# SamsungLabs/Metis

Measured on AMD Instinct MI355X. Metric: best_plan_iter_time_ms, lower is better.
Workload: dtype bf16; 1 GPU; model=gpt3-2.7b, global_batch=16, seq_len=2048, parallelism=dp1_tp1_pp1, microbatch=16

## Files before the change

### metis_amd/ops/hip/bindings.cpp

```cpp
#include <torch/extension.h>

#include <vector>

std::vector<torch::Tensor> layernorm_fwd(
    torch::Tensor x, torch::Tensor gamma, torch::Tensor beta, double eps);
std::vector<torch::Tensor> layernorm_bwd(
    torch::Tensor dy, torch::Tensor x, torch::Tensor gamma,
    torch::Tensor mean, torch::Tensor rstd);
std::vector<torch::Tensor> bias_residual_layernorm_fwd(
    torch::Tensor y, torch::Tensor bias, torch::Tensor residual,
    torch::Tensor gamma, torch::Tensor beta, double eps);
torch::Tensor bias_residual_add(
    torch::Tensor y, torch::Tensor bias, torch::Tensor residual);
std::vector<torch::Tensor> layernorm_bwd_add(
    torch::Tensor dy, torch::Tensor dres, torch::Tensor x, torch::Tensor gamma,
    torch::Tensor mean, torch::Tensor rstd, bool want_colsum);
std::vector<torch::Tensor> gelu_tanh_bwd_bgrad(torch::Tensor h, torch::Tensor da);
void adamw_step(
    torch::Tensor master, torch::Tensor model, torch::Tensor grad,
    torch::Tensor m, torch::Tensor v,
    double lr, double beta1, double beta2, double eps,
    double weight_decay, long step, double grad_scale);
torch::Tensor attn_decode(
    torch::Tensor q, torch::Tensor k, torch::Tensor v, double scale);
torch::Tensor attn_decode_ragged(
    torch::Tensor q, torch::Tensor k, torch::Tensor v, torch::Tensor kv_lens,
    double scale, long num_splits);
torch::Tensor attn_decode_ragged_fp8(
    torch::Tensor q, torch::Tensor k8, torch::Tensor v8,
    torch::Tensor k_scale, torch::Tensor v_scale, torch::Tensor kv_lens,
    double scale, long num_splits);
void kv_quant_store(
    torch::Tensor k, torch::Tensor v, torch::Tensor k8, torch::Tensor v8,
    torch::Tensor k_scale, torch::Tensor v_scale, torch::Tensor slots,
    torch::Tensor pos);
torch::Tensor w8_linear(
    torch::Tensor x, torch::Tensor w8, torch::Tensor scale,
    c10::optional<torch::Tensor> bias, long num_splits);
long w8_linear_auto_splits(long N, long K);
torch::Tensor ce_row_max(torch::Tensor logits);
torch::Tensor ce_row_sumexp(torch::Tensor logits, torch::Tensor m);
std::vector<torch::Tensor> qkv_rope_split(
    torch::Tensor qkv, long nq, long nkv, long head_dim,
    torch::Tensor cos_t, torch::Tensor sin_t);
torch::Tensor qkv_rope_split_bwd(
    torch::Tensor dq, torch::Tensor dk, torch::Tensor dv, long head_dim,
    torch::Tensor cos_t, torch::Tensor sin_t);
torch::Tensor lt_fp8_matmul(
    torch::Tensor x, torch::Tensor w,
    torch::Tensor scale_x, torch::Tensor scale_w);
std::vector<torch::Tensor> lt_fc1_forward(
    torch::Tensor x, torch::Tensor w, torch::Tensor bias);
std::vector<torch::Tensor> lt_matmul_dgelu_bgrad(
    torch::Tensor dy, torch::Tensor w2, torch::Tensor pre_gelu);
std::vector<torch::Tensor> attn_fwd(
    torch::Tensor q, torch::Tensor k, torch::Tensor v, double scale);
std::vector<torch::Tensor> attn_bwd(
    torch::Tensor q, torch::Tensor k, torch::Tensor v,
    torch::Tensor d_o, torch::Tensor lse, torch::Tensor delta,
    double scale);
torch::Tensor attn_bwd_delta(torch::Tensor o, torch::Tensor d_o);
std::vector<torch::Tensor> attn_fwd_packed(
    torch::Tensor qkv, long H, long Hkv, long D, double scale);
torch::Tensor attn_bwd_delta_packed(torch::Tensor o, torch::Tensor d_o, long H);
torch::Tensor attn_bwd_packed(
    torch::Tensor qkv, torch::Tensor d_o, torch::Tensor lse, torch::Tensor delta,
    long H, long Hkv, long D, double scale);
torch::Tensor gemm_bf16(
    torch::Tensor a, torch::Tensor b_nk, c10::optional<torch::Tensor> bias,
    long epilogue);
torch::Tensor mfma_tile_probe(torch::Tensor a, torch::Tensor b);
torch::Tensor gemm8_bf16(torch::Tensor x, torch::Tensor w);
std::vector<torch::Tensor> rmsnorm_fwd(
    torch::Tensor x, torch::Tensor gamma, double eps);
std::vector<torch::Tensor> rmsnorm_bwd(
    torch::Tensor dy, torch::Tensor x, torch::Tensor gamma, torch::Tensor rstd);
torch::Tensor rope_apply(
    torch::Tensor x, torch::Tensor cos_t, torch::Tensor sin_t, bool backward);
torch::Tensor swiglu_fwd(torch::Tensor a, torch::Tensor b);
std::vector<torch::Tensor> swiglu_bwd(
    torch::Tensor dy, torch::Tensor a, torch::Tensor b);
std::vector<torch::Tensor> cross_entropy_fwd(
    torch::Tensor logits, torch::Tensor labels);
torch::Tensor cross_entropy_bwd(
    torch::Tensor logits, torch::Tensor labels, torch::Tensor lse,
    torch::Tensor grad_scale);
std::vector<torch::Tensor> qkv_split_transpose(
    torch::Tensor qkv, long nq, long nkv, long head_dim);
torch::Tensor qkv_split_transpose_bwd(
    torch::Tensor dq, torch::Tensor dk, torch::Tensor dv, long head_dim);
torch::Tensor heads_merge(torch::Tensor x);
torch::Tensor heads_unmerge(torch::Tensor y, long H);
torch::Tensor tr16_probe(long stride_elems);
torch::Tensor lt_linear_dgrad_tn(torch::Tensor dy, torch::Tensor wt);
torch::Tensor lt_linear_dgrad(torch::Tensor dy, torch::Tensor w, long algo);
torch::Tensor lt_linear_wgrad(torch::Tensor dy, torch::Tensor x, long algo);
long lt_version();
std::vector<long> lt_supported_algos(
    const std::string& op, long M, long N, long K);
long lt_heuristic_algo(const std::string& op, long M, long N, long K);
long lt_wgrad_bgradb_algos(long M, long N, long K);
torch::Tensor transpose_bf16(torch::Tensor w);
void transpose_bf16_out(torch::Tensor w, torch::Tensor wt);

PYBIND11_MODULE(TORCH_EXTENSION_NAME, m) {
    m.def("layernorm_fwd", &layernorm_fwd,
          "fused LayerNorm forward (bf16, fp32 stats)");
    m.def("layernorm_bwd", &layernorm_bwd,
          "fused LayerNorm backward (dx + dgamma/dbeta)");
    m.def("bias_residual_layernorm_fwd", &bias_residual_layernorm_fwd,
          "x = residual + (y + bias) with both bf16 roundings, then "
          "LayerNorm(x) -> (x, z, mean, rstd)");
    m.def("bias_residual_add", &bias_residual_add,
          "x = residual + (y + bias) with both bf16 roundings");
    m.def("layernorm_bwd_add", &layernorm_bwd_add,
          "LayerNorm backward with a residual gradient folded in -> "
          "(g = dres + dx, dgamma, dbeta, colsum of g in fp32 or empty)");
    m.def("gelu_tanh_bwd_bgrad", &gelu_tanh_bwd_bgrad,
          "tanh-GeLU backward -> (dh bf16, dbias = column sums of dh, fp32)");
    m.def("adamw_step", &adamw_step, "fused AdamW step");
    m.def("attn_fwd", &attn_fwd,
          "flash attention forward (causal, GQA) -> (O, LSE)");
    m.def("attn_bwd", &attn_bwd,
          "flash attention backward -> (dQ, dK_per_head, dV_per_head)");
    m.def("attn_bwd_delta", &attn_bwd_delta,
          "rowsum(dO * O) in fp32 -> [B,H,S] (contiguous bf16 inputs)");
    m.def("attn_fwd_packed", &attn_fwd_packed,
          "flash attention forward on qkv [B,S,(H+2Hkv)D] in place "
          "(H == Hkv) -> (O [B,S,H*D], LSE [B,H,S])");
    m.def("attn_bwd_delta_packed", &attn_bwd_delta_packed,
          "rowsum(dO * O) of [B,S,H*D] operands in fp32 -> [B,H,S]");
    m.def("attn_bwd_packed", &attn_bwd_packed,
          "flash attention backward on qkv in place -> dqkv [B,S,(H+2Hkv)D]");
    m.def("gemm_bf16", &gemm_bf16,
          "MFMA bf16 GEMM A[M,K] @ B[N,K]^T with fused epilogue "
          "(0=none, 1=bias, 2=bias+gelu)");
    m.def("gemm8_bf16", &gemm8_bf16,
          "256^2-tile 2-buffer glds bf16 GEMM x[M,K] @ w[N,K]^T");
    m.def("mfma_tile_probe", &mfma_tile_probe,
          "single-wave 16x16x32 MFMA layout probe");
    m.def("rmsnorm_fwd", &rmsnorm_fwd, "fused RMSNorm forward");
    m.def("rmsnorm_bwd", &rmsnorm_bwd, "fused RMSNorm backward");
    m.def("rope_apply", &rope_apply, "rotary embedding (fwd/bwd by flag)");
    m.def("swiglu_fwd", &swiglu_fwd, "fused silu(a)*b");
    m.def("swiglu_bwd", &swiglu_bwd, "fused SwiGLU backward");
    m.def("cross_entropy_fwd", &cross_entropy_fwd,
          "fused CE over bf16 logits -> (per-row loss, lse)");
    m.def("cross_entropy_bwd", &cross_entropy_bwd,
          "fused CE backward -> bf16 dlogits");
    m.def("qkv_split_transpose", &qkv_split_transpose,
          "[B,S,(nq+2nkv)D] -> q/k/v [B,h,S,D] in one pass");
    m.def("qkv_split_transpose_bwd", &qkv_split_transpose_bwd,
          "dq/dk/dv -> fused dqkv layout");
    m.def("heads_merge", &heads_merge, "[B,H,S,D] -> [B,S,H*D]");
    m.def("heads_unmerge", &heads_unmerge, "[B,S,H*D] -> [B,H,S,D]");
    m.def("attn_decode", &attn_decode,
          "single-query attention over cached K/V (GQA, online softmax)");
    m.def("attn_decode_ragged", &attn_decode_ragged,
          "ragged split-S single-query attention over a padded K/V cache "
          "(per-row kv_lens, strided views, GQA group per workgroup)",
          pybind11::arg("q"), pybind11::arg("k"), pybind11::arg("v"),
          pybind11::arg("kv_lens"), pybind11::arg("scale"),
          pybind11::arg("num_splits") = 0);
    m.def("attn_decode_ragged_fp8", &attn_decode_ragged_fp8,
          "ragged split-S single-query attention over an fp8 (e4m3fn) K/V "
          "cache with one fp32 scale per (batch row, kv head, position)",
          pybind11::arg("q"), pybind11::arg("k8"), pybind11::arg("v8"),
          pybind11::arg("k_scale"), pybind11::arg("v_scale"),
          pybind11::arg("kv_lens"), pybind11::arg("scale"),
          pybind11::arg("num_splits") = 0);
    m.def("kv_quant_store", &kv_quant_store,
          "quantise bf16 K/V rows [N,Hkv,T,D] to e4m3fn + per-row fp32 scale "
          "and store them at position pos[n] + t of cache row slots[n]",
          pybind11::arg("k"), pybind11::arg("v"), pybind11::arg("k8"),
          pybind11::arg("v8"), pybind11::arg("k_scale"),
          pybind11::arg("v_scale"), pybind11::arg("slots"),
          pybind11::arg("pos"));
    m.def("w8_linear", &w8_linear,
          "fp8 (e4m3fn) weight-only linear for 1 <= M <= 16 bf16 rows: "
          "scale[n] * (x @ w8^T) + bias, fp32 accumulation, split-K",
          pybind11::arg("x"), pybind11::arg("w8"), pybind11::arg("scale"),
          pybind11::arg("bias") = pybind11::none(),
          pybind11::arg("num_splits") = 0);
    m.def("w8_linear_auto_splits", &w8_linear_auto_splits,
          "split count w8_linear picks for num_splits = 0 (from N and K only)");
    m.def("ce_row_max", &ce_row_max, "per-row max of bf16 logits (fp32)");
    m.def("ce_row_sumexp", &ce_row_sumexp,
          "per-row sum(exp(x - m)) of bf16 logits (fp32)");
    m.def("qkv_rope_split", &qkv_rope_split,
          "fused QKV relayout + RoPE (neox) forward");
    m.def("qkv_rope_split_bwd", &qkv_rope_split_bwd,
          "fused QKV relayout + RoPE backward gather");
    m.def("lt_fp8_matmul", &lt_fp8_matmul,
          "fp8 e4m3 GEMM with per-tensor scales, bf16 out");
    m.def("lt_fc1_forward", &lt_fc1_forward,
          "hipblaslt GEMM with GELU_AUX_BIAS epilogue (fc1 fused)");
    m.def("lt_matmul_dgelu_bgrad", &lt_matmul_dgelu_bgrad,
          "hipblaslt GEMM with DGELU_BGRAD epilogue (fc2 data grad fused)");
    m.def("lt_linear_dgrad_tn", &lt_linear_dgrad_tn,
          "dx [M,K] = dy [M,N] @ wt [K,N]^T (hipBLASLt TN route)");
    m.def("lt_linear_dgrad", &lt_linear_dgrad,
          "dx [M,K] = dy [M,N] @ w [N,K]; algo = solution index or -1");
    m.def("lt_linear_wgrad", &lt_linear_wgrad,
          "dw [N,K] = dy [M,N]^T @ x [M,K]; algo = solution index or -1");
    m.def("lt_version", &lt_version, "hipblasLtGetVersion");
    m.def("lt_supported_algos", &lt_supported_algos,
          "supported solution indices for op (dgrad_tn|dgrad|wgrad) at M,N,K");
    m.def("lt_heuristic_algo", &lt_heuristic_algo,
          "solution index of the heuristic's first choice");
    m.def("lt_wgrad_bgradb_algos", &lt_wgrad_bgradb_algos,
          "number of weight-gradient algorithms with the BGRADB epilogue");
    m.def("transpose_bf16", &transpose_bf16, "wt [C,R] = w [R,C]^T");
    m.def("transpose_bf16_out", &transpose_bf16_out,
          "transpose into an existing [C,R] buffer");
    m.def("tr16_probe", &tr16_probe,
          "ds_read_b64_tr_b16 lane-semantics probe (debug)");
}
```

### metis_amd/ops/hip/lt_gemm.cpp

```cpp

#include <torch/extension.h>

#include <hipblaslt/hipblaslt.h>
#include <hipblaslt/hipblaslt-ext.hpp>

#include <c10/hip/HIPStream.h>

#include <climits>
#include <mutex>
#include <stdexcept>
#include <string>
#include <unordered_map>
#include <vector>

namespace {

#define LT_CHECK(expr)                                                        \
    do {                                                                      \
        hipblasStatus_t s_ = (expr);                                          \
        TORCH_CHECK(s_ == HIPBLAS_STATUS_SUCCESS, "hipblaslt error ",         \
                    (int)s_, " at ", #expr);                                  \
    } while (0)

hipblasLtHandle_t lt_handle() {
    static hipblasLtHandle_t handle = [] {
        hipblasLtHandle_t h;
        LT_CHECK(hipblasLtCreate(&h));
        return h;
    }();
    return handle;
}

constexpr size_t kWorkspaceBytes = 64ull << 20;

torch::Tensor workspace(const torch::TensorOptions& opt) {
    static torch::Tensor ws;
    if (!ws.defined() || ws.numel() < (long)kWorkspaceBytes)
        ws = torch::empty({(long)kWorkspaceBytes},
                          opt.dtype(torch::kUInt8));
    return ws;
}

struct LtPlan {
    hipblasLtMatmulDesc_t desc{};
    hipblasLtMatrixLayout_t a{}, b{}, d{};
    hipblasLtMatmulAlgo_t algo{};
    bool has_algo = false;
};

std::unordered_map<std::string, LtPlan>& plan_cache() {
    static std::unordered_map<std::string, LtPlan> cache;
    return cache;
}
std::mutex cache_mutex;

void destroy_plan(LtPlan& plan) {
    if (plan.a) hipblasLtMatrixLayoutDestroy(plan.a);
    if (plan.b) hipblasLtMatrixLayoutDestroy(plan.b);
    if (plan.d) hipblasLtMatrixLayoutDestroy(plan.d);
    if (plan.desc) hipblasLtMatmulDescDestroy(plan.desc);
    plan = LtPlan{};
}

LtPlan& get_plan(hipblasLtEpilogue_t epi, bool transa, bool transb, long m,
                 long n, long k, int algo_index, const void* bias,
                 const void* aux, long aux_ld) {
    std::lock_guard<std::mutex> lock(cache_mutex);
    std::string key = std::to_string((int)epi) + (transa ? "t" : "n") +
                      (transb ? "t" : "n") + "_" + std::to_string(m) + "_" +
                      std::to_string(n) + "_" + std::to_string(k) + "_" +
                      std::to_string(algo_index);
    auto it = plan_cache().find(key);
    if (it != plan_cache().end()) return it->second;

    LtPlan plan;
    LT_CHECK(hipblasLtMatmulDescCreate(&plan.desc, HIPBLAS_COMPUTE_32F,
                                       HIP_R_32F));
    hipblasOperation_t opA = transa ? HIPBLAS_OP_T : HIPBLAS_OP_N;
    hipblasOperation_t opB = transb ? HIPBLAS_OP_T : HIPBLAS_OP_N;
    LT_CHECK(hipblasLtMatmulDescSetAttribute(
        plan.desc, HIPBLASLT_MATMUL_DESC_TRANSA, &opA, sizeof(opA)));
    LT_CHECK(hipblasLtMatmulDescSetAttribute(
        plan.desc, HIPBLASLT_MATMUL_DESC_TRANSB, &opB, sizeof(opB)));
    LT_CHECK(hipblasLtMatmulDescSetAttribute(
        plan.desc, HIPBLASLT_MATMUL_DESC_EPILOGUE, &epi, sizeof(epi)));
    if (bias != nullptr)
        LT_CHECK(hipblasLtMatmulDescSetAttribute(
            plan.desc, HIPBLASLT_MATMUL_DESC_BIAS_POINTER, &bias,
            sizeof(bias)));
    if (aux != nullptr) {
        LT_CHECK(hipblasLtMatmulDescSetAttribute(
            plan.desc, HIPBLASLT_MATMUL_DESC_EPILOGUE_AUX_POINTER, &aux,
            sizeof(aux)));
        LT_CHECK(hipblasLtMatmulDescSetAttribute(
            plan.desc, HIPBLASLT_MATMUL_DESC_EPILOGUE_AUX_LD, &aux_ld,
            sizeof(aux_ld)));
    }

    if (transa)
        LT_CHECK(hipblasLtMatrixLayoutCreate(&plan.a, HIP_R_16BF, k, m, k));
    else
        LT_CHECK(hipblasLtMatrixLayoutCreate(&plan.a, HIP_R_16BF, m, k, m));
    if (transb)
        LT_CHECK(hipblasLtMatrixLayoutCreate(&plan.b, HIP_R_16BF, n, k, n));
    else
        LT_CHECK(hipblasLtMatrixLayoutCreate(&plan.b, HIP_R_16BF, k, n, k));
    LT_CHECK(hipblasLtMatrixLayoutCreate(&plan.d, HIP_R_16BF, m, n, m));

    if (algo_index >= 0) {
        std::vector<int> index{algo_index};
        std::vector<hipblasLtMatmulHeuristicResult_t> results;
        hipblasStatus_t st =
            hipblaslt_ext::getAlgosFromIndex(lt_handle(), index, results);
        float alpha = 1.0f, beta = 0.0f;
        size_t ws_needed = 0;
        if (st == HIPBLAS_STATUS_SUCCESS && !results.empty())
            st = hipblaslt_ext::matmulIsAlgoSupported(
                lt_handle(), plan.desc, &alpha, plan.a, plan.b, &beta, plan.d,
                plan.d, results[0].algo, ws_needed);
        else if (st == HIPBLAS_STATUS_SUCCESS)
            st = HIPBLAS_STATUS_INVALID_VALUE;
        if (st != HIPBLAS_STATUS_SUCCESS || ws_needed > kWorkspaceBytes) {
            destroy_plan(plan);
            TORCH_CHECK(false, "hipblaslt: algorithm index ", algo_index,
                        " is not supported for op ", (transa ? "T" : "N"),
                        (transb ? "T" : "N"), " m=", m, " n=", n, " k=", k,
                        " (status ", (int)st, ", workspace ", ws_needed, ")");
        }
        plan.algo = results[0].algo;
        plan.has_algo = true;
        return plan_cache().emplace(key, plan).first->second;
    }

    hipblasLtMatmulPreference_t pref;
    LT_CHECK(hipblasLtMatmulPreferenceCreate(&pref));
    uint64_t ws_bytes = kWorkspaceBytes;
    LT_CHECK(hipblasLtMatmulPreferenceSetAttribute(
        pref, HIPBLASLT_MATMUL_PREF_MAX_WORKSPACE_BYTES, &ws_bytes,
        sizeof(ws_bytes)));
    hipblasLtMatmulHeuristicResult_t result{};
    int found = 0;
    LT_CHECK(hipblasLtMatmulAlgoGetHeuristic(
        lt_handle(), plan.desc, plan.a, plan.b, plan.d, plan.d, pref, 1,
        &result, &found));
    LT_CHECK(hipblasLtMatmulPreferenceDestroy(pref));
    if (found <= 0) destroy_plan(plan);
    TORCH_CHECK(found > 0, "hipblaslt: no algorithm for epilogue ", (int)epi,
                " at m=", m, " n=", n, " k=", k);
    plan.algo = result.algo;
    plan.has_algo = true;
    return plan_cache().emplace(key, plan).first->second;
}

void run_matmul(LtPlan& plan, const void* wA, const void* xB, void* outD,
                const void* bias, const void* aux, long aux_ld,
                hipblasLtEpilogue_t epi, long M, long N, long K,
                const torch::TensorOptions& opt) {
    if (bias != nullptr)
        LT_CHECK(hipblasLtMatmulDescSetAttribute(
            plan.desc, HIPBLASLT_MATMUL_DESC_BIAS_POINTER, &bias,
            sizeof(bias)));
    if (aux != nullptr) {
        LT_CHECK(hipblasLtMatmulDescSetAttribute(
            plan.desc, HIPBLASLT_MATMUL_DESC_EPILOGUE_AUX_POINTER, &aux,
            sizeof(aux)));
        LT_CHECK(hipblasLtMatmulDescSetAttribute(
            plan.desc, HIPBLASLT_MATMUL_DESC_EPILOGUE_AUX_LD, &aux_ld,
            sizeof(aux_ld)));
    }
    float alpha = 1.0f, beta = 0.0f;
    auto ws = workspace(opt);
    auto stream = c10::hip::getCurrentHIPStream().stream();
    LT_CHECK(hipblasLtMatmul(
        lt_handle(), plan.desc, &alpha, wA, plan.a, xB, plan.b, &beta, outD,
        plan.d, outD, plan.d, plan.has_algo ? &plan.algo : nullptr,
        ws.data_ptr(), kWorkspaceBytes, stream));
}

}

std::vector<torch::Tensor> lt_fc1_forward(torch::Tensor x, torch::Tensor w,
                                          torch::Tensor bias) {
    TORCH_CHECK(x.is_cuda() && x.dtype() == torch::kBFloat16);
    TORCH_CHECK(x.dim() == 2 && w.dim() == 2 && x.size(1) == w.size(1),
                "x [M,K], w [N,K]");
    auto xc = x.contiguous(), wc = w.contiguous(), bc = bias.contiguous();
    const long M = x.size(0), K = x.size(1), N = w.size(0);
    auto y = torch::empty({M, N}, x.options());
    auto aux = torch::empty({M, N}, x.options());

    auto& plan = get_plan(HIPBLASLT_EPILOGUE_GELU_AUX_BIAS, true, false, N, M,
                          K, -1, bc.data_ptr(), aux.data_ptr(), N);
    run_matmul(plan, wc.data_ptr(), xc.data_ptr(), y.data_ptr(),
               bc.data_ptr(), aux.data_ptr(), N,
               HIPBLASLT_EPILOGUE_GELU_AUX_BIAS, M, N, K, x.options());
    return {y, aux};
}

std::vector<torch::Tensor> lt_matmul_dgelu_bgrad(torch::Tensor dy,
                                                 torch::Tensor w2,
                                                 torch::Tensor pre_gelu) {
    TORCH_CHECK(dy.is_cuda() && dy.dtype() == torch::kBFloat16);
    TORCH_CHECK(dy.dim() == 2 && w2.dim() == 2 && dy.size(1) == w2.size(0),
                "dy [M,H], w2 [H,N]");
    auto dyc = dy.contiguous(), w2c = w2.contiguous();
    auto auxc = pre_gelu.contiguous();
    const long M = dy.size(0), H = dy.size(1), N = w2.size(1);
    TORCH_CHECK(pre_gelu.size(0) == M && pre_gelu.size(1) == N);
    auto dpre = torch::empty({M, N}, dy.options());
    auto dbias = torch::empty({N}, dy.options());

    auto& plan = get_plan(HIPBLASLT_EPILOGUE_DGELU_BGRAD, false, false, N, M,
                          H, -1, dbias.data_ptr(), auxc.data_ptr(), N);
    run_matmul(plan, w2c.data_ptr(), dyc.data_ptr(), dpre.data_ptr(),
               dbias.data_ptr(), auxc.data_ptr(), N,
               HIPBLASLT_EPILOGUE_DGELU_BGRAD, M, N, H, dy.options());
    return {dpre, dbias};
}

torch::Tensor lt_fp8_matmul(torch::Tensor x, torch::Tensor w,
                            torch::Tensor scale_x, torch::Tensor scale_w) {
    TORCH_CHECK(x.is_cuda() && x.dtype() == torch::kFloat8_e4m3fn);
    TORCH_CHECK(w.dtype() == torch::kFloat8_e4m3fn);
    TORCH_CHECK(x.dim() == 2 && w.dim() == 2 && x.size(1) == w.size(1));
    TORCH_CHECK(scale_x.dtype() == torch::kFloat32 && scale_x.numel() == 1);
    auto xc = x.contiguous(), wc = w.contiguous();
    const long M = x.size(0), K = x.size(1), N = w.size(0);
    auto y = torch::empty({M, N},
                          x.options().dtype(torch::kBFloat16));

    std::lock_guard<std::mutex> lock(cache_mutex);
    std::string key = "fp8_" + std::to_string(M) + "_" + std::to_string(N) +
                      "_" + std::to_string(K);
    auto it = plan_cache().find(key);
    if (it == plan_cache().end()) {
        LtPlan plan;
        LT_CHECK(hipblasLtMatmulDescCreate(&plan.desc, HIPBLAS_COMPUTE_32F,
                                           HIP_R_32F));
        hipblasOperation_t opT = HIPBLAS_OP_T, opN = HIPBLAS_OP_N;
        LT_CHECK(hipblasLtMatmulDescSetAttribute(
            plan.desc, HIPBLASLT_MATMUL_DESC_TRANSA, &opT, sizeof(opT)));
        LT_CHECK(hipblasLtMatmulDescSetAttribute(
            plan.desc, HIPBLASLT_MATMUL_DESC_TRANSB, &opN, sizeof(opN)));
        LT_CHECK(hipblasLtMatrixLayoutCreate(&plan.a, HIP_R_8F_E4M3, K, N, K));
        LT_CHECK(hipblasLtMatrixLayoutCreate(&plan.b, HIP_R_8F_E4M3, K, M, K));
        LT_CHECK(hipblasLtMatrixLayoutCreate(&plan.d, HIP_R_16BF, N, M, N));
        hipblasLtMatmulPreference_t pref;
        LT_CHECK(hipblasLtMatmulPreferenceCreate(&pref));
        uint64_t ws_bytes = kWorkspaceBytes;
        LT_CHECK(hipblasLtMatmulPreferenceSetAttribute(
            pref, HIPBLASLT_MATMUL_PREF_MAX_WORKSPACE_BYTES, &ws_bytes,
            sizeof(ws_bytes)));
        hipblasLtMatmulHeuristicResult_t result{};
        int found = 0;
        LT_CHECK(hipblasLtMatmulAlgoGetHeuristic(
            lt_handle(), plan.desc, plan.a, plan.b, plan.d, plan.d, pref, 1,
            &result, &found));
        LT_CHECK(hipblasLtMatmulPreferenceDestroy(pref));
        TORCH_CHECK(found > 0, "hipblaslt: no fp8 algorithm at M=", M,
                    " N=", N, " K=", K);
        plan.algo = result.algo;
        plan.has_algo = true;
        it = plan_cache().emplace(key, plan).first;
    }
    LtPlan& plan = it->second;
    const void* sa = scale_w.data_ptr();
    const void* sb = scale_x.data_ptr();
    LT_CHECK(hipblasLtMatmulDescSetAttribute(
        plan.desc, HIPBLASLT_MATMUL_DESC_A_SCALE_POINTER, &sa, sizeof(sa)));
    LT_CHECK(hipblasLtMatmulDescSetAttribute(
        plan.desc, HIPBLASLT_MATMUL_DESC_B_SCALE_POINTER, &sb, sizeof(sb)));
    float alpha = 1.0f, beta = 0.0f;
    auto ws = workspace(y.options());
    auto stream = c10::hip::getCurrentHIPStream().stream();
    LT_CHECK(hipblasLtMatmul(
        lt_handle(), plan.desc, &alpha, wc.data_ptr(), plan.a, xc.data_ptr(),
        plan.b, &beta, y.data_ptr(), plan.d, y.data_ptr(), plan.d,
        &plan.algo, ws.data_ptr(), kWorkspaceBytes, stream));
    return y;
}

namespace {

enum class BwdOp { DgradTN, Dgrad, Wgrad };

BwdOp parse_bwd_op(const std::string& op) {
    if (op == "dgrad_tn") return BwdOp::DgradTN;
    if (op == "dgrad") return BwdOp::Dgrad;
    if (op == "wgrad") return BwdOp::Wgrad;
    TORCH_CHECK(false, "unknown op '", op, "' (dgrad_tn, dgrad, wgrad)");
}

struct BwdProblem {
    bool transa, transb;
    long m, n, k;
};

BwdProblem bwd_problem(BwdOp op, long M, long N, long K) {
    switch (op) {
    case BwdOp::DgradTN: return {true, false, K, M, N};
    case BwdOp::Dgrad:   return {false, false, K, M, N};
    default:             return {false, true, K, N, M};
    }
}

void check_operand(const torch::Tensor& t, const char* name) {
    TORCH_CHECK(t.is_cuda(), name, " must be a CUDA tensor");
    TORCH_CHECK(t.dtype() == torch::kBFloat16, name, " must be bf16");
    TORCH_CHECK(t.dim() == 2, name, " must be 2-d");
    TORCH_CHECK(t.is_contiguous(), name, " must be contiguous");
    TORCH_CHECK(t.numel() > 0, name, " must not be empty");
    TORCH_CHECK(reinterpret_cast<uintptr_t>(t.data_ptr()) % 16 == 0, name,
                " must be 16-byte aligned");
}

void check_pair(const torch::Tensor& a, const char* an,
                const torch::Tensor& b, const char* bn) {
    check_operand(a, an);
    check_operand(b, bn);
    TORCH_CHECK(a.device() == b.device(), an, " and ", bn,
                " must be on one device");
}

torch::Tensor run_bwd(BwdOp op, long M, long N, long K, long algo,
                      const torch::Tensor& colA, const torch::Tensor& colB,
                      long out_rows, long out_cols) {
    TORCH_CHECK(algo >= -1 && algo <= INT_MAX, "bad algorithm index ", algo);
    BwdProblem p = bwd_problem(op, M, N, K);
    auto& plan = get_plan(HIPBLASLT_EPILOGUE_DEFAULT, p.transa, p.transb, p.m,
                          p.n, p.k, (int)algo, nullptr, nullptr, 0);
    auto out = torch::empty({out_rows, out_cols}, colA.options());
    run_matmul(plan, colA.data_ptr(), colB.data_ptr(), out.data_ptr(), nullptr,
               nullptr, 0, HIPBLASLT_EPILOGUE_DEFAULT, M, N, K,
               colA.options());
    return out;
}

}

torch::Tensor lt_linear_dgrad_tn(torch::Tensor dy, torch::Tensor wt) {
    check_pair(dy, "dy", wt, "wt");
    TORCH_CHECK(dy.size(1) == wt.size(1), "dy [M,N], wt [K,N]: inner sizes ",
                dy.size(1), " and ", wt.size(1), " differ");
    const long M = dy.size(0), N = dy.size(1), K = wt.size(0);
    return run_bwd(BwdOp::DgradTN, M, N, K, -1, wt, dy, M, K);
}

torch::Tensor lt_linear_dgrad(torch::Tensor dy, torch::Tensor w, long algo) {
    check_pair(dy, "dy", w, "w");
    TORCH_CHECK(dy.size(1) == w.size(0), "dy [M,N], w [N,K]: inner sizes ",
                dy.size(1), " and ", w.size(0), " differ");
    const long M = dy.size(0), N = dy.size(1), K = w.size(1);
    return run_bwd(BwdOp::Dgrad, M, N, K, algo, w, dy, M, K);
}

torch::Tensor lt_linear_wgrad(torch::Tensor dy, torch::Tensor x, long algo) {
    check_pair(dy, "dy", x, "x");
    TORCH_CHECK(dy.size(0) == x.size(0), "dy [M,N], x [M,K]: inner sizes ",
                dy.size(0), " and ", x.size(0), " differ");
    const long M = dy.size(0), N = dy.size(1), K = x.size(1);
    return run_bwd(BwdOp::Wgrad, M, N, K, algo, x, dy, N, K);
}


long lt_version() {
    int v = 0;
    LT_CHECK(hipblasLtGetVersion(lt_handle(), &v));
    return v;
}

std::vector<long> lt_supported_algos(const std::string& op, long M, long N,
                                     long K) {
    BwdProblem p = bwd_problem(parse_bwd_op(op), M, N, K);
    std::vector<hipblasLtMatmulHeuristicResult_t> all;
    LT_CHECK(hipblaslt_ext::getAllAlgos(
        lt_handle(), hipblaslt_ext::GemmType::HIPBLASLT_GEMM,
        p.transa ? HIPBLAS_OP_T : HIPBLAS_OP_N,
        p.transb ? HIPBLAS_OP_T : HIPBLAS_OP_N, HIP_R_16BF, HIP_R_16BF,
        HIP_R_16BF, HIP_R_16BF, HIPBLAS_COMPUTE_32F, all));
    LtPlan* plan;
    {
        plan = &get_plan(HIPBLASLT_EPILOGUE_DEFAULT, p.transa, p.transb, p.m,
                         p.n, p.k, -1, nullptr, nullptr, 0);
    }
    std::vector<long> out;
    float alpha = 1.0f, beta = 0.0f;
    for (auto& r : all) {
        size_t ws_needed = 0;
        hipblasStatus_t st = hipblaslt_ext::matmulIsAlgoSupported(
            lt_handle(), plan->desc, &alpha, plan->a, plan->b, &beta, plan->d,
            plan->d, r.algo, ws_needed);
        if (st == HIPBLAS_STATUS_SUCCESS && ws_needed <= kWorkspaceBytes)
            out.push_back(hipblaslt_ext::getIndexFromAlgo(r.algo));
    }
    return out;
}

long lt_heuristic_algo(const std::string& op, long M, long N, long K) {
    BwdProblem p = bwd_problem(parse_bwd_op(op), M, N, K);
    auto& plan = get_plan(HIPBLASLT_EPILOGUE_DEFAULT, p.transa, p.transb, p.m,
                          p.n, p.k, -1, nullptr, nullptr, 0);
    return hipblaslt_ext::getIndexFromAlgo(plan.algo);
}

long lt_wgrad_bgradb_algos(long M, long N, long K) {
    BwdProblem p = bwd_problem(BwdOp::Wgrad, M, N, K);
    LtPlan plan;
    LT_CHECK(hipblasLtMatmulDescCreate(&plan.desc, HIPBLAS_COMPUTE_32F,
                                       HIP_R_32F));
    hipblasOperation_t opA = HIPBLAS_OP_N, opB = HIPBLAS_OP_T;
    hipblasLtEpilogue_t epi = HIPBLASLT_EPILOGUE_BGRADB;
    LT_CHECK(hipblasLtMatmulDescSetAttribute(
        plan.desc, HIPBLASLT_MATMUL_DESC_TRANSA, &opA, sizeof(opA)));
    LT_CHECK(hipblasLtMatmulDescSetAttribute(
        plan.desc, HIPBLASLT_MATMUL_DESC_TRANSB, &opB, sizeof(opB)));
    LT_CHECK(hipblasLtMatmulDescSetAttribute(
        plan.desc, HIPBLASLT_MATMUL_DESC_EPILOGUE, &epi, sizeof(epi)));
    LT_CHECK(hipblasLtMatrixLayoutCreate(&plan.a, HIP_R_16BF, p.m, p.k, p.m));
    LT_CHECK(hipblasLtMatrixLayoutCreate(&plan.b, HIP_R_16BF, p.n, p.k, p.n));
    LT_CHECK(hipblasLtMatrixLayoutCreate(&plan.d, HIP_R_16BF, p.m, p.n, p.m));
    hipblasLtMatmulPreference_t pref;
    LT_CHECK(hipblasLtMatmulPreferenceCreate(&pref));
    uint64_t ws_bytes = kWorkspaceBytes;
    LT_CHECK(hipblasLtMatmulPreferenceSetAttribute(
        pref, HIPBLASLT_MATMUL_PREF_MAX_WORKSPACE_BYTES, &ws_bytes,
        sizeof(ws_bytes)));
    hipblasLtMatmulHeuristicResult_t results[8];
    int found = 0;
    hipblasStatus_t st = hipblasLtMatmulAlgoGetHeuristic(
        lt_handle(), plan.desc, plan.a, plan.b, plan.d, plan.d, pref, 8,
        results, &found);
    hipblasLtMatmulPreferenceDestroy(pref);
    destroy_plan(plan);
    return st == HIPBLAS_STATUS_SUCCESS ? found : 0;
}
```

### metis_amd/ops/linear.py

```python

from __future__ import annotations

import json
import logging
import os
from typing import Dict, Optional, Tuple

import torch
import torch.nn.functional as F

from metis_amd import ops as _ops

_log = logging.getLogger(__name__)

TABLE_PATH = os.path.join(
    os.path.dirname(os.path.dirname(os.path.dirname(os.path.abspath(__file__)))),
    "profiles", "mi355x", "gemm_algos.json")

OPS = ("dgrad", "wgrad")
ROUTES = {"dgrad": ("aten", "lt", "lt_tn"), "wgrad": ("aten", "lt")}

Key = Tuple[str, int, int, int]


class GemmTable:

    def __init__(self, lt_version: int, device: str,
                 entries: Dict[Key, Tuple[str, int]]):
        self.lt_version = lt_version
        self.device = device
        self.entries = entries

    @classmethod
    def empty(cls) -> "GemmTable":
        return cls(-1, "", {})

    @classmethod
    def parse(cls, obj) -> "GemmTable":
        if not isinstance(obj, dict):
            raise ValueError("table is not an object")
        version, device = obj.get("hipblaslt_version"), obj.get("device")
        if not _is_int(version) or not isinstance(device, str):
            raise ValueError("header needs hipblaslt_version (int) and device")
        raw = obj.get("entries")
        if not isinstance(raw, list):
            raise ValueError("entries is not a list")
        entries: Dict[Key, Tuple[str, int]] = {}
        for e in raw:
            if not isinstance(e, dict):
                raise ValueError("entry is not an object")
            op, route, algo = e.get("op"), e.get("route"), e.get("algo", -1)
            dims = (e.get("M"), e.get("N"), e.get("K"))
            if op not in OPS or route not in ROUTES[op]:
                raise ValueError(f"bad op/route {op!r}/{route!r}")
            if not all(_is_int(d) and d > 0 for d in dims):
                raise ValueError(f"bad shape {dims!r}")
            if not _is_int(algo) or algo < -1:
                raise ValueError(f"bad algo {algo!r}")
            key = (op,) + dims
            if key in entries:
                raise ValueError(f"duplicate entry {key!r}")
            entries[key] = (route, algo)
        return cls(version, device, entries)

    def matches(self, lt_version: int, device: str) -> bool:
        return self.lt_version == lt_version and self.device == device

    def lookup(self, op: str, M: int, N: int, K: int) -> Tuple[str, int]:
        return self.entries.get((op, M, N, K), ("aten", -1))


def _is_int(v) -> bool:
    return isinstance(v, int) and not isinstance(v, bool)


def load_table(path: str) -> GemmTable:
    try:
        with open(path) as f:
            return GemmTable.parse(json.load(f))
    except (OSError, ValueError) as e:
        _log.warning("gemm table %s not used (%s): linear backward GEMMs "
                     "take the aten route", path, e)
        return GemmTable.empty()


def resolve_table(table: GemmTable, lt_version: int, device: str) -> GemmTable:
    if not table.entries or table.matches(lt_version, device):
        return table
    _log.warning(
        "gemm table was tuned for hipBLASLt %s on %r, this is %s on %r: "
        "linear backward GEMMs take the aten route",
        table.lt_version, table.device, lt_version, device)
    return GemmTable.empty()


_FILE_TABLE = load_table(os.environ.get("METIS_GEMM_TABLE") or TABLE_PATH)
_ACTIVE: Optional[GemmTable] = None


def device_id() -> str:
    p = torch.cuda.get_device_properties(torch.cuda.current_device())
    return f"{p.gcnArchName.split(':')[0]}-{p.multi_processor_count}cu"


def _active_table() -> GemmTable:
    global _ACTIVE
    if _ACTIVE is None:
        ext = _ops.require_extension()
        _ACTIVE = resolve_table(_FILE_TABLE, int(ext.lt_version()),
                                device_id())
    return _ACTIVE


class use_table:

    def __init__(self, table: GemmTable):
        self.table = table

    def __enter__(self):
        global _ACTIVE
        self._saved = _ACTIVE
        _ACTIVE = self.table
        return self.table

    def __exit__(self, *exc):
        global _ACTIVE
        _ACTIVE = self._saved
        return False


def enabled() -> bool:
    return os.environ.get("METIS_LT_BWD", "1") != "0"


_epoch = 0
transpose_refreshes = 0


def bump_epoch() -> None:
    global _epoch
    _epoch += 1


def _stamp(weight: torch.Tensor):
    return (_epoch, weight._version, weight.data_ptr(),
            getattr(weight, "_metis_fwd_count", 0))


def transposed_weight(weight: torch.Tensor) -> torch.Tensor:
    global transpose_refreshes
    ext = _ops.require_extension()
    stamp = _stamp(weight)
    cached = getattr(weight, "_metis_wt", None)
    if cached is not None and cached[0] == stamp:
        return cached[1]
    w = weight.detach()
    if (cached is not None and cached[1].device == w.device
            and cached[1].shape == (w.size(1), w.size(0))):
        wt = cached[1]
    else:
        wt = torch.empty(w.size(1), w.size(0), dtype=w.dtype, device=w.device)
    ext.transpose_bf16_out(w, wt)
    weight._metis_wt = (stamp, wt)
    transpose_refreshes += 1
    return wt


def _lt_ok(*tensors: torch.Tensor) -> bool:
    if not all(t.is_cuda and t.dtype == torch.bfloat16 for t in tensors):
        return False
    return not torch.cuda.is_current_stream_capturing()


def _lt_operand(t: torch.Tensor) -> torch.Tensor:
    t = t.contiguous()
    return t if t.data_ptr() % 16 == 0 else t.clone()


class _Linear(torch.autograd.Function):
    @staticmethod
    def forward(ctx, x, weight, bias):
        ctx.save_for_backward(x, weight)
        ctx.has_bias = bias is not None
        weight._metis_fwd_count = getattr(weight, "_metis_fwd_count", 0) + 1
        ctx.weight_ref = weight
        return F.linear(x, weight, bias)

    @staticmethod
    def backward(ctx, dy):
        x, w = ctx.saved_tensors
        N, K = w.shape
        dy2 = dy.reshape(-1, N)
        x2 = x.reshape(-1, K)
        M = dy2.size(0)
        lt = _lt_ok(dy2, x2, w)
        table = _active_table() if lt else None
        dx = dw = db = None

        if ctx.needs_input_grad[0]:
            route, algo = table.lookup("dgrad", M, N, K) if lt else ("aten", -1)
            if route == "lt_tn" and N % 8 == 0 and K % 8 == 0:
                wt = transposed_weight(ctx.weight_ref)
                dx2 = _ops.require_extension().lt_linear_dgrad_tn(
                    _lt_operand(dy2), wt)
            elif route == "lt":
                dx2 = _ops.require_extension().lt_linear_dgrad(
                    _lt_operand(dy2), _lt_operand(w), algo)
            else:
                dx2 = dy2 @ w
            dx = dx2.view(x.shape)
        if ctx.needs_input_grad[1]:
            route, algo = table.lookup("wgrad", M, N, K) if lt else ("aten", -1)
            if route == "lt":
                dw = _ops.require_extension().lt_linear_wgrad(
                    _lt_operand(dy2), _lt_operand(x2), algo)
            else:
                dw = dy2.t() @ x2
        if ctx.has_bias and ctx.needs_input_grad[2]:
            db = dy2.sum(0, keepdim=True).view(N)
        return dx, dw, db


def linear(x: torch.Tensor, weight: torch.Tensor,
           bias: Optional[torch.Tensor] = None) -> torch.Tensor:
    if not enabled():
        return F.linear(x, weight, bias)
    return _Linear.apply(x, weight, bias)
```

Baseline: 675.1 ms.

## Add transposed-operand wgrad GEMM routes selectable from the tuning table

Adds four new hipBLASLt weight-gradient variants that take a pre-transposed dy and/or x (NN, TT, TN layouts) and route wgrad through them when the GEMM table selects one. Operands are transposed into per-stream scratch buffers before the GEMM. The aim is to reach faster hipBLASLt kernels for the wgrad shapes, at the cost of extra transpose kernels and scratch memory. Whether anything changes depends on the profile table listing the new routes, and the diff does not update that table.

```diff
diff --git a/metis_amd/ops/hip/bindings.cpp b/metis_amd/ops/hip/bindings.cpp
--- a/metis_amd/ops/hip/bindings.cpp
+++ b/metis_amd/ops/hip/bindings.cpp
@@ -95,6 +95,13 @@
 torch::Tensor lt_linear_dgrad_tn(torch::Tensor dy, torch::Tensor wt);
 torch::Tensor lt_linear_dgrad(torch::Tensor dy, torch::Tensor w, long algo);
 torch::Tensor lt_linear_wgrad(torch::Tensor dy, torch::Tensor x, long algo);
+torch::Tensor lt_linear_wgrad_dyt(torch::Tensor dyt, torch::Tensor x,
+                                  long algo);
+torch::Tensor lt_linear_wgrad_xt(torch::Tensor dy, torch::Tensor xt, long algo);
+torch::Tensor lt_linear_wgrad_xt_nn(torch::Tensor dy, torch::Tensor xt,
+                                    long algo);
+torch::Tensor lt_linear_wgrad_tn(torch::Tensor dyt, torch::Tensor xt,
+                                 long algo);
 long lt_version();
 std::vector<long> lt_supported_algos(
     const std::string& op, long M, long N, long K);
@@ -203,9 +210,18 @@
           "dx [M,K] = dy [M,N] @ w [N,K]; algo = solution index or -1");
     m.def("lt_linear_wgrad", &lt_linear_wgrad,
           "dw [N,K] = dy [M,N]^T @ x [M,K]; algo = solution index or -1");
+    m.def("lt_linear_wgrad_dyt", &lt_linear_wgrad_dyt,
+          "dw [N,K] = dyT [N,M] @ x [M,K] (NN); algo = solution index or -1");
+    m.def("lt_linear_wgrad_xt", &lt_linear_wgrad_xt,
+          "dw [N,K] = dy [M,N]^T @ xT [K,M]^T (TT); algo as above");
+    m.def("lt_linear_wgrad_xt_nn", &lt_linear_wgrad_xt_nn,
+          "dwT [K,N] = xT [K,M] @ dy [M,N] (NN); algo as above");
+    m.def("lt_linear_wgrad_tn", &lt_linear_wgrad_tn,
+          "dw [N,K] = dyT [N,M] @ xT [K,M]^T (TN); algo as above");
     m.def("lt_version", &lt_version, "hipblasLtGetVersion");
     m.def("lt_supported_algos", &lt_supported_algos,
-          "supported solution indices for op (dgrad_tn|dgrad|wgrad) at M,N,K");
+          "supported solution indices for op (dgrad_tn|dgrad|wgrad|wgrad_dyt|"
+          "wgrad_xt|wgrad_xt_nn|wgrad_tn) at M,N,K");
     m.def("lt_heuristic_algo", &lt_heuristic_algo,
           "solution index of the heuristic's first choice");
     m.def("lt_wgrad_bgradb_algos", &lt_wgrad_bgradb_algos,
diff --git a/metis_amd/ops/hip/lt_gemm.cpp b/metis_amd/ops/hip/lt_gemm.cpp
--- a/metis_amd/ops/hip/lt_gemm.cpp
+++ b/metis_amd/ops/hip/lt_gemm.cpp
@@ -282,13 +282,20 @@
 
 namespace {
 
-enum class BwdOp { DgradTN, Dgrad, Wgrad };
+enum class BwdOp {
+    DgradTN, Dgrad, Wgrad, WgradDyT, WgradXT, WgradXTNN, WgradTN
+};
 
 BwdOp parse_bwd_op(const std::string& op) {
     if (op == "dgrad_tn") return BwdOp::DgradTN;
     if (op == "dgrad") return BwdOp::Dgrad;
     if (op == "wgrad") return BwdOp::Wgrad;
-    TORCH_CHECK(false, "unknown op '", op, "' (dgrad_tn, dgrad, wgrad)");
+    if (op == "wgrad_dyt") return BwdOp::WgradDyT;
+    if (op == "wgrad_xt") return BwdOp::WgradXT;
+    if (op == "wgrad_xt_nn") return BwdOp::WgradXTNN;
+    if (op == "wgrad_tn") return BwdOp::WgradTN;
+    TORCH_CHECK(false, "unknown op '", op, "' (dgrad_tn, dgrad, wgrad, "
+                "wgrad_dyt, wgrad_xt, wgrad_xt_nn, wgrad_tn)");
 }
 
 struct BwdProblem {
@@ -300,6 +307,10 @@
     switch (op) {
     case BwdOp::DgradTN: return {true, false, K, M, N};
     case BwdOp::Dgrad:   return {false, false, K, M, N};
+    case BwdOp::WgradDyT:  return {false, false, K, N, M};
+    case BwdOp::WgradXT:   return {true, true, K, N, M};
+    case BwdOp::WgradXTNN: return {false, false, N, K, M};
+    case BwdOp::WgradTN:   return {true, false, K, N, M};
     default:             return {false, true, K, N, M};
     }
 }
@@ -360,6 +371,42 @@
                 dy.size(0), " and ", x.size(0), " differ");
     const long M = dy.size(0), N = dy.size(1), K = x.size(1);
     return run_bwd(BwdOp::Wgrad, M, N, K, algo, x, dy, N, K);
+}
+
+torch::Tensor lt_linear_wgrad_dyt(torch::Tensor dyt, torch::Tensor x,
+                                  long algo) {
+    check_pair(dyt, "dyT", x, "x");
+    TORCH_CHECK(dyt.size(1) == x.size(0), "dyT [N,M], x [M,K]: inner sizes ",
+                dyt.size(1), " and ", x.size(0), " differ");
+    const long M = x.size(0), N = dyt.size(0), K = x.size(1);
+    return run_bwd(BwdOp::WgradDyT, M, N, K, algo, x, dyt, N, K);
+}
+
+torch::Tensor lt_linear_wgrad_xt(torch::Tensor dy, torch::Tensor xt,
+                                 long algo) {
+    check_pair(dy, "dy", xt, "xT");
+    TORCH_CHECK(dy.size(0) == xt.size(1), "dy [M,N], xT [K,M]: inner sizes ",
+                dy.size(0), " and ", xt.size(1), " differ");
+    const long M = dy.size(0), N = dy.size(1), K = xt.size(0);
+    return run_bwd(BwdOp::WgradXT, M, N, K, algo, xt, dy, N, K);
+}
+
+torch::Tensor lt_linear_wgrad_xt_nn(torch::Tensor dy, torch::Tensor xt,
+                                    long algo) {
+    check_pair(dy, "dy", xt, "xT");
+    TORCH_CHECK(dy.size(0) == xt.size(1), "dy [M,N], xT [K,M]: inner sizes ",
+                dy.size(0), " and ", xt.size(1), " differ");
+    const long M = dy.size(0), N = dy.size(1), K = xt.size(0);
+    return run_bwd(BwdOp::WgradXTNN, M, N, K, algo, dy, xt, K, N);
+}
+
+torch::Tensor lt_linear_wgrad_tn(torch::Tensor dyt, torch::Tensor xt,
+                                 long algo) {
+    check_pair(dyt, "dyT", xt, "xT");
+    TORCH_CHECK(dyt.size(1) == xt.size(1), "dyT [N,M], xT [K,M]: inner sizes ",
+                dyt.size(1), " and ", xt.size(1), " differ");
+    const long M = dyt.size(1), N = dyt.size(0), K = xt.size(0);
+    return run_bwd(BwdOp::WgradTN, M, N, K, algo, xt, dyt, N, K);
 }
 
 
diff --git a/metis_amd/ops/linear.py b/metis_amd/ops/linear.py
--- a/metis_amd/ops/linear.py
+++ b/metis_amd/ops/linear.py
@@ -18,7 +18,8 @@
     "profiles", "mi355x", "gemm_algos.json")
 
 OPS = ("dgrad", "wgrad")
-ROUTES = {"dgrad": ("aten", "lt", "lt_tn"), "wgrad": ("aten", "lt")}
+ROUTES = {"dgrad": ("aten", "lt", "lt_tn"),
+          "wgrad": ("aten", "lt", "lt_dyt", "lt_xt", "lt_xt_nn", "lt_dyt_xt")}
 
 Key = Tuple[str, int, int, int]
 
@@ -177,6 +178,42 @@
     return t if t.data_ptr() % 16 == 0 else t.clone()
 
 
+_scratch: Dict[Tuple[int, int, int], torch.Tensor] = {}
+
+
+def _transposed_scratch(t: torch.Tensor, slot: int) -> torch.Tensor:
+    key = (t.device.index, torch.cuda.current_stream(t.device).cuda_stream,
+           slot)
+    buf = _scratch.get(key)
+    if buf is None or buf.numel() < t.numel():
+        del buf
+        _scratch.pop(key, None)
+        buf = _scratch[key] = torch.empty(t.numel(), dtype=t.dtype,
+                                          device=t.device)
+    out = buf[:t.numel()].view(t.size(1), t.size(0))
+    _ops.require_extension().transpose_bf16_out(t, out)
+    return out
+
+
+def _wgrad(route: str, algo: int, dy2: torch.Tensor,
+           x2: torch.Tensor) -> torch.Tensor:
+    ext = _ops.require_extension()
+    dy2, x2 = _lt_operand(dy2), _lt_operand(x2)
+    if route == "lt":
+        return ext.lt_linear_wgrad(dy2, x2, algo)
+    if route == "lt_dyt":
+        return ext.lt_linear_wgrad_dyt(_transposed_scratch(dy2, 0), x2, algo)
+    if route == "lt_xt":
+        return ext.lt_linear_wgrad_xt(dy2, _transposed_scratch(x2, 0), algo)
+    if route == "lt_xt_nn":
+        return ext.transpose_bf16(
+            ext.lt_linear_wgrad_xt_nn(dy2, _transposed_scratch(x2, 0), algo))
+    if route == "lt_dyt_xt":
+        return ext.lt_linear_wgrad_tn(_transposed_scratch(dy2, 0),
+                                      _transposed_scratch(x2, 1), algo)
+    raise ValueError(f"unknown wgrad route {route!r}")
+
+
 class _Linear(torch.autograd.Function):
     @staticmethod
     def forward(ctx, x, weight, bias):
@@ -211,9 +248,9 @@
             dx = dx2.view(x.shape)
         if ctx.needs_input_grad[1]:
             route, algo = table.lookup("wgrad", M, N, K) if lt else ("aten", -1)
-            if route == "lt":
-                dw = _ops.require_extension().lt_linear_wgrad(
-                    _lt_operand(dy2), _lt_operand(x2), algo)
+            if route == "lt" or (route != "aten" and M % 8 == 0
+                                 and N % 8 == 0 and K % 8 == 0):
+                dw = _wgrad(route, algo, dy2, x2)
             else:
                 dw = dy2.t() @ x2
         if ctx.has_bias and ctx.needs_input_grad[2]:
```

Measured after the change: 642.2 ms, median of 6. -4.9%, faster.
